# CERALIVE/ceracoder

Measured on AMD Instinct MI355X. Metric: 1080p H.264 encoded frames/sec per GPU, higher is better.
Workload: dtype u8

## Files before the change

ceracoder_amd/csrc/k_motion.hip:

```cpp
#include "kernels_common.hpp"

#ifndef ME_MBS
#define ME_MBS 4
#endif
#define ME_WQ (ME_MBS + 2)
#define ME_ROWS 50
#define ME_STRIDE 53
#define ME_K 5

DEV unsigned long long qsad(unsigned lo, unsigned hi, unsigned cur, unsigned long long acc) {
    unsigned long long src = ((unsigned long long)hi << 32) | lo;
    return __builtin_amdgcn_qsad_pk_u16_u8(src, cur, acc);
}
DEV int mv_bits(int v) {
    int a = iabs(v);
    return a == 0 ? 1 : 7 + 2 * (31 - __clz(a));
}
DEV int med3(int a, int b, int c) {
    const int lo = a < b ? a : b, hi = a < b ? b : a;
    return c < lo ? lo : (c > hi ? hi : c);
}
struct fpred_t { int px, py, sx, sy; };
DEV fpred_t field_pred(const imv_t *__restrict__ f, int mbw, int mx, int my, bool top) {
    const bool avA = mx > 0, avB = top, avC = top && mx + 1 < mbw, avD = mx > 0 && top, hasC = avC || avD;
// ... 146 lines not shown
#endif
#ifdef ME_DBG_NOSURF
    if (active && acc[0] == 0x123456789ull) {
#else
    if (active) {
#endif
        uint16_t *sf = ctx->surf + (size_t)(my * mbw + mx) * SURF_U16 + 4 * dxg;
#pragma unroll
        for (int d = 0; d < ME_K; d++) stg64(sf + (ME_K * g + d) * SURF_COLS, make_uint2((unsigned)acc[d], (unsigned)(acc[d] >> 32)));
    }
#ifdef ME_DBG_NOSEL
    const unsigned best = ((((unsigned)acc[0] ^ (unsigned)acc[4]) & 0x0FFFu) << 12) | 0x410u;
#else
    const unsigned best = select_min<true>(acc, g, dxg, active, ctx->me_range, ctx->lambda, 0, 0, 0, 0);
#endif
    if (lane == 0 && mx < mbw) store_imv(&ctx->imv_a[my * mbw + mx], best, ctx->lambda, 0, 0, 0, 0);
    tl_last(ctx, 1);
}

__global__ __launch_bounds__(256) void me_select_kernel(const frame_ctx_t cv, int mb0, int mb1, const imv_t *__restrict__ in, imv_t *__restrict__ out,
                                                        const imv_t *__restrict__ prev, int mode) {
    const frame_ctx_t *__restrict__ ctx = &cv;
    const int mbw = ctx->mbw;
    const int lane = threadIdx.x & 63, wave = __builtin_amdgcn_readfirstlane(threadIdx.x >> 6);
    const int mbn = mb0 + xcd_remap(blockIdx.x, gridDim.x) * 4 + wave;
    if (mbn >= mb1) return;
    const int my = mbn / mbw, mx = mbn - my * mbw;
    const fpred_t fp = field_pred(in, mbw, mx, my, row_has_top(ctx, my));
    const int px = fp.px >> 2, py = fp.py >> 2, sx = fp.sx >> 2, sy = fp.sy >> 2;
    if (mode) {
        fpred_t fq = {0, 0, 0, 0};
        if (mode == 2) fq = field_pred(prev, mbw, mx, my, row_has_top(ctx, my));
        if (px == (fq.px >> 2) && py == (fq.py >> 2) && sx == (fq.sx >> 2) && sy == (fq.sy >> 2)) {
            if (lane == 0) stg64(&out[mbn], ldg64(&in[mbn]));
            return;
        }
    }
    const bool active = lane < 63;
    const int g = active ? lane / 9 : 0, dxg = active ? lane % 9 : 0;
    unsigned long long acc[ME_K];
    const uint16_t *sf = ctx->surf + (size_t)mbn * SURF_U16 + 4 * dxg;
#pragma unroll
    for (int d = 0; d < ME_K; d++) { const uint2 v = ldg64(sf + (ME_K * g + d) * SURF_COLS); acc[d] = ((unsigned long long)v.y << 32) | v.x; }
    const unsigned best = select_min(acc, g, dxg, active, ctx->me_range, ctx->lambda, px, py, sx, sy);
    if (lane == 0) store_imv(&out[mbn], best, ctx->lambda, px, py, sx, sy);
}

#ifndef SEL_SPW
#define SEL_SPW 8
#endif
__global__ __launch_bounds__(256) void me_select_sparse_kernel(const frame_ctx_t cv, int mb0, int mb1, const imv_t *__restrict__ in, imv_t *__restrict__ out, const imv_t *__restrict__ prev) {
    const frame_ctx_t *__restrict__ ctx = &cv;
    const int mbw = ctx->mbw;
    const int lane = threadIdx.x & 63, wave = __builtin_amdgcn_readfirstlane(threadIdx.x >> 6);
    const int base = mb0 + ((int)blockIdx.x * 4 + wave) * SEL_SPW;
    if (base >= mb1) return;
    const int mine = base + (lane < SEL_SPW ? lane : 0);
    const bool have = lane < SEL_SPW && mine < mb1;
    const int mbn_l = have ? mine : base, my_l = mbn_l / mbw, mx_l = mbn_l - my_l * mbw;
    const bool top_l = row_has_top(ctx, my_l);
    const fpred_t fp = field_pred(in, mbw, mx_l, my_l, top_l), fq = field_pred(prev, mbw, mx_l, my_l, top_l);
    const int px = fp.px >> 2, py = fp.py >> 2, sx = fp.sx >> 2, sy = fp.sy >> 2;
    const bool same = px == (fq.px >> 2) && py == (fq.py >> 2) && sx == (fq.sx >> 2) && sy == (fq.sy >> 2);
    if (have && same) stg64(&out[mbn_l], ldg64(&in[mbn_l]));
    unsigned todo = (unsigned)(__ballot(have && !same) & ((1ull << SEL_SPW) - 1ull));
    const bool active = lane < 63;
    const int g = active ? lane / 9 : 0, dxg = active ? lane % 9 : 0;
    while (todo) {
        const int j = __builtin_ctz(todo);
        todo &= todo - 1;
        const int mbn = base + j;
        const int jpx = __builtin_amdgcn_readlane(px, j), jpy = __builtin_amdgcn_readlane(py, j), jsx = __builtin_amdgcn_readlane(sx, j), jsy = __builtin_amdgcn_readlane(sy, j);
        unsigned long long acc[ME_K];
        const uint16_t *sf = ctx->surf + (size_t)mbn * SURF_U16 + 4 * dxg;
#pragma unroll
        for (int d = 0; d < ME_K; d++) { const uint2 v = ldg64(sf + (ME_K * g + d) * SURF_COLS); acc[d] = ((unsigned long long)v.y << 32) | v.x; }
        const unsigned best = select_min(acc, g, dxg, active, ctx->me_range, ctx->lambda, jpx, jpy, jsx, jsy);
        if (lane == 0) store_imv(&out[mbn], best, ctx->lambda, jpx, jpy, jsx, jsy);
    }
}

#define SP_GS 24
#define SP_PS 20
struct sp_lds {
    uint8_t G[23 * SP_GS];
    int16_t H1[18 * SP_GS];
    uint8_t b[19 * SP_PS];
    uint8_t h[18 * SP_GS];
    uint8_t j[18 * SP_PS];
    uint8_t pad[16];
};
typedef short sp_s2 __attribute__((ext_vector_type(2)));
DEV sp_s2 as_s2(unsigned v) { return __builtin_bit_cast(sp_s2, v); }
DEV unsigned as_u(sp_s2 v) { return __builtin_bit_cast(unsigned, v); }
DEV sp_s2 bytes_lo(unsigned w) { return as_s2(__builtin_amdgcn_perm(0u, w, 0x0c010c00u)); }
DEV sp_s2 bytes_hi(unsigned w) { return as_s2(__builtin_amdgcn_perm(0u, w, 0x0c030c02u)); }
DEV sp_s2 clip255_s2(sp_s2 v) { return __builtin_elementwise_min(__builtin_elementwise_max(v, (sp_s2)(0)), (sp_s2)(255)); }
DEV sp_s2 pair_s2(int a, int b) { return as_s2(__builtin_amdgcn_perm((unsigned)b, (unsigned)a, 0x05040100u)); }
DEV unsigned pack_s2(sp_s2 lo, sp_s2 hi) { return __builtin_amdgcn_perm(as_u(hi), as_u(lo), 0x06040200u); }
DEV unsigned clip_pack4(int a, int b, int c, int d) { return pack_s2(clip255_s2(pair_s2(a, b)), clip255_s2(pair_s2(c, d))); }
DEV int mvq_bits(int q) {
    unsigned k = q > 0 ? (unsigned)(2 * q - 1) : (unsigned)(-2 * q);
    return 2 * (31 - __clz((int)(k + 1))) + 1;
}
DEV unsigned lds4(const uint8_t *plane, int o) {
    const unsigned *w = (const unsigned *)(plane + (o & ~3));
    return __builtin_amdgcn_alignbyte(w[1], w[0], (unsigned)(o & 3));
}
DEV unsigned sp_sample4(const sp_lds *L, int X, int Y, int fx, int fy) {
#define SG(x, y) lds4(L->G, ((y) + 2) * SP_GS + (x) + 2)
#define SB(x, y) lds4(L->b, (y) * SP_PS + (x))
#define SH(x, y) lds4(L->h, (y) * SP_GS + (x) + 2)
#define SJ(x, y) lds4(L->j, (y) * SP_PS + (x))
    if (fy == 0) {
        if (fx == 0) return SG(X, Y);
        return fx == 2 ? SB(X, Y) : fx == 1 ? avg4(SG(X, Y), SB(X, Y)) : avg4(SG(X + 1, Y), SB(X, Y));
    }
    if (fx == 0) return fy == 2 ? SH(X, Y) : fy == 1 ? avg4(SG(X, Y), SH(X, Y)) : avg4(SG(X, Y + 1), SH(X, Y));
    if ((fx & 1) && (fy & 1)) return avg4(fy == 1 ? SB(X, Y) : SB(X, Y + 1), fx == 1 ? SH(X, Y) : SH(X + 1, Y));
    if (fx == 2 && fy == 2) return SJ(X, Y);
    if (fx == 2) return avg4(fy == 1 ? SB(X, Y) : SB(X, Y + 1), SJ(X, Y));
    return avg4(fx == 1 ? SH(X, Y) : SH(X + 1, Y), SJ(X, Y));
#undef SG
#undef SB
#undef SH
#undef SJ
}
DEV void sp_planes(sp_lds *L, const int lane) {
    if (lane < 54) {
        const int d = lane % 6, seg = lane / 6;
        sp_s2 lo[7], hi[7];
#pragma unroll
        for (int r = 0; r < 7; r++) {
            const unsigned w = *(const unsigned *)&L->G[(2 * seg + r) * SP_GS + 4 * d];
            lo[r] = bytes_lo(w); hi[r] = bytes_hi(w);
        }
#pragma unroll
        for (int t = 0; t < 2; t++) {
            const sp_s2 vl = (lo[t + 2] + lo[t + 3]) * (sp_s2)(20) - (lo[t + 1] + lo[t + 4]) * (sp_s2)(5) + (lo[t] + lo[t + 5]);
            const sp_s2 vh = (hi[t + 2] + hi[t + 3]) * (sp_s2)(20) - (hi[t + 1] + hi[t + 4]) * (sp_s2)(5) + (hi[t] + hi[t + 5]);
            const int R = 2 * seg + t;
            unsigned *o = (unsigned *)&L->H1[R * SP_GS + 4 * d];
            o[0] = as_u(vl); o[1] = as_u(vh);
            *(unsigned *)&L->h[R * SP_GS + 4 * d] = pack_s2(clip255_s2((vl + (sp_s2)(16)) >> (sp_s2)(5)), clip255_s2((vh + (sp_s2)(16)) >> (sp_s2)(5)));
        }
    }
#pragma unroll
    for (int it = 0; it < 2; it++) {
        const int i = lane + 64 * it;
        if (i < 19 * 5) {
            const int R = i / 5, g = i - R * 5;
            const unsigned *gw = (const unsigned *)&L->G[(R + 2) * SP_GS + 4 * g];
            const unsigned d0 = gw[0] ^ 0x80808080u, d1 = gw[1] ^ 0x80808080u, d2 = gw[2] ^ 0x80808080u;
            int o[4];
#pragma unroll
            for (int k = 0; k < 4; k++) {
                const unsigned w0 = k ? __builtin_amdgcn_alignbyte(d1, d0, (unsigned)k) : d0, w1 = k ? __builtin_amdgcn_alignbyte(d2, d1, (unsigned)k) : d1;
                const int v = __builtin_amdgcn_sdot4((int)w0, 0x1414FB01, __builtin_amdgcn_sdot4((int)w1, 0x000001FB, 4096, false), false);
                o[k] = (v + 16) >> 5;
            }
            *(unsigned *)&L->b[R * SP_PS + 4 * g] = clip_pack4(o[0], o[1], o[2], o[3]);
        }
    }
    WAVE_SYNC();
#pragma unroll
    for (int it = 0; it < 2; it++) {
        const int i = lane + 64 * it;
        if (i < 18 * 5) {
            const int R = i / 5, g = i - R * 5;
            const unsigned *hw = (const unsigned *)&L->H1[R * SP_GS + 4 * g];
            const unsigned p0 = hw[0], p1 = hw[1], p2 = hw[2], p3 = hw[3], p4 = hw[4];
            const unsigned q0 = __builtin_amdgcn_alignbyte(p1, p0, 2u), q1 = __builtin_amdgcn_alignbyte(p2, p1, 2u),
                           q2 = __builtin_amdgcn_alignbyte(p3, p2, 2u), q3 = __builtin_amdgcn_alignbyte(p4, p3, 2u);
// ... 12 lines not shown
    const int mbw = ctx->mbw, mbh = ctx->mbh, stride = ctx->stride, W = mbw * 16, H = mbh * 16;
    const int lane = threadIdx.x & 63, wave = __builtin_amdgcn_readfirstlane(threadIdx.x >> 6);
    int mbn = mb0 + blockIdx.x * 4 + wave;
    const bool ok = mbn < mb1;
    if (!ok) mbn = mb1 - 1;
    const int my = mbn / mbw, mx = mbn - my * mbw, x0 = mx * 16, y0 = my * 16;
    sp_lds *L = &LD[wave];
    const mb_info_t info = ld_mbinfo(&ctx->mbi[mbn]);
    const int ix = x0 + (info.mvx >> 2), iy = y0 + (info.mvy >> 2);
    const uint8_t *__restrict__ ref = ctx->ref_y;
    if (ix - 3 >= 0 && iy - 3 >= 0 && ((ix - 3) & ~3) + 28 <= W && iy + 19 < H) {
        const int a = (ix - 3) & 3;
        const uint8_t *base = ref + (size_t)(iy - 3) * stride + ((ix - 3) & ~3);
        for (int i = lane; i < 23 * 6; i += 64) {
            const int r = i / 6, d = i - r * 6;
            const unsigned w0 = ldg32(base + (size_t)r * stride + 4 * d), w1 = ldg32(base + (size_t)r * stride + 4 * d + 4);
            *(unsigned *)&L->G[r * SP_GS + 4 * d] = __builtin_amdgcn_alignbyte(w1, w0, (unsigned)a);
        }
    } else
        for (int i = lane; i < 23 * 23; i += 64) {
            int r = i / 23, c = i - r * 23;
            int yy = clip3(0, H - 1, iy - 3 + r), xx = clip3(0, W - 1, ix - 3 + c);
            L->G[r * SP_GS + c] = (uint8_t)ldg8(ref + (size_t)yy * stride + xx);
        }
    const int pr = lane >> 2, pc = (lane & 3) * 4;
    unsigned curw;
    {
        int sy = y0 + pr;
        sy = sy < ctx->vis_h ? sy : ctx->vis_h - 1;
        curw = ldg32(ctx->src_y + (size_t)sy * ctx->src_stride + x0 + pc);
    }
    WAVE_SYNC();
    sp_planes(L, lane);
    const int lambda = ctx->lambda;
    int bqx = info.mvx, bqy = info.mvy;
    unsigned best = info.cost;
#pragma unroll 1
    for (int step = 2; step >= 1; step--) {
        const int cqx = bqx, cqy = bqy;
        unsigned acc[4] = {0, 0, 0, 0};
#pragma unroll
        for (int c8 = 0; c8 < 8; c8++) {
            const int k = c8 < 4 ? c8 : c8 + 1;
            const int qx = cqx + (k % 3 - 1) * step, qy = cqy + (k / 3 - 1) * step;
            const int ox = qx - info.mvx, oy = qy - info.mvy;
            const int X = 1 + (ox >> 2) + pc, Y = 1 + (oy >> 2) + pr;
            const unsigned sad = __builtin_amdgcn_sad_u8(curw, sp_sample4(L, X, Y, ox & 3, oy & 3), 0u);
            acc[c8 >> 1] |= sad << (16 * (c8 & 1));
        }
#pragma unroll
        for (int q = 0; q < 4; q++) {
            acc[q] = (unsigned)wave64_sum((int)acc[q]);
        }
#pragma unroll
        for (int c8 = 0; c8 < 8; c8++) {
            const int k = c8 < 4 ? c8 : c8 + 1;
            const int qx = cqx + (k % 3 - 1) * step, qy = cqy + (k / 3 - 1) * step;
            const unsigned sad = (acc[c8 >> 1] >> (16 * (c8 & 1))) & 0xFFFFu;
            const unsigned cost = sad + (unsigned)(lambda * (mvq_bits(qx) + mvq_bits(qy)));
            if (cost < best) { best = cost; bqx = qx; bqy = qy; }
        }
    }
    if (lane == 0 && ok) {
        mb_info_t *mb = &ctx->mbi[mbn];
        stg32(&mb->mvx, ((unsigned)(uint16_t)bqx) | ((unsigned)(uint16_t)bqy << 16));
        stg32(&mb->cost, best);
    }
}

DEV int dec_score(unsigned M) { return dec_score_mask(M); }
DEV int row_or4(int v) {
    v |= __builtin_amdgcn_update_dpp(0, v, 0x128, 0xF, 0xF, false);
    v |= __builtin_amdgcn_update_dpp(0, v, 0x124, 0xF, 0xF, false);
    return v;
}
DEV unsigned ref_word4(const uint8_t *__restrict__ ref, int stride, int W, int H, int x, int y, bool inside) {
    if (inside) {
        const uint8_t *b = ref + (size_t)y * stride + (x & ~3);
        return __builtin_amdgcn_alignbyte(ldg32(b + 4), ldg32(b), (unsigned)(x & 3));
    }
    const uint8_t *r = ref + (size_t)clip3(0, H - 1, y) * stride;
    return pack4((int)ldg8(r + clip3(0, W - 1, x)), (int)ldg8(r + clip3(0, W - 1, x + 1)), (int)ldg8(r + clip3(0, W - 1, x + 2)), (int)ldg8(r + clip3(0, W - 1, x + 3)));
}
DEV void chroma_pred4(const frame_ctx_t *__restrict__ ctx, int lane, int x0, int y0, int W, int H, int mvx, int mvy, int *pd) {
    const int stride = ctx->stride;
    const int py = (lane >> 2) & 3, cby = (lane >> 4) & 1, c = (lane >> 1) & 1, cbx = lane & 1;
    const int cx0 = x0 >> 1, cy0 = y0 >> 1, cw = W >> 1, ch = H >> 1;
    const int cy = cby * 4 + py, cxb = cbx * 4;
    const int xi = mvx >> 3, yi = mvy >> 3, xf = mvx & 7, yf = mvy & 7;
    const uint8_t *__restrict__ rf = ctx->ref_uv;
    int A[5], B[5];
    if (cx0 + xi >= 0 && cx0 + xi + 9 <= cw && cy0 + yi >= 0 && cy0 + yi + 9 <= ch) {
        const int o = 2 * (cx0 + cxb + xi) + c, a = o & 3;
        const uint8_t *r0 = rf + (size_t)(cy0 + cy + yi) * stride + (o & ~3), *r1 = r0 + stride;
        const unsigned a0 = ldg32(r0), a1 = ldg32(r0 + 4), a2 = ldg32(r0 + 8), b0 = ldg32(r1), b1 = ldg32(r1 + 4), b2 = ldg32(r1 + 8);
        const unsigned sa0 = __builtin_amdgcn_alignbyte(a1, a0, (unsigned)a), sa1 = __builtin_amdgcn_alignbyte(a2, a1, (unsigned)a);
        const unsigned sb0 = __builtin_amdgcn_alignbyte(b1, b0, (unsigned)a), sb1 = __builtin_amdgcn_alignbyte(b2, b1, (unsigned)a);
        A[0] = byte_of(sa0, 0); A[1] = byte_of(sa0, 2); A[2] = byte_of(sa1, 0); A[3] = byte_of(sa1, 2); A[4] = (int)((a2 >> (8 * a)) & 255);
        B[0] = byte_of(sb0, 0); B[1] = byte_of(sb0, 2); B[2] = byte_of(sb1, 0); B[3] = byte_of(sb1, 2); B[4] = (int)((b2 >> (8 * a)) & 255);
    } else {
        const int ya = clip3(0, ch - 1, cy0 + cy + yi), yb = clip3(0, ch - 1, cy0 + cy + yi + 1);
#pragma unroll
        for (int i = 0; i < 5; i++) {
            const int xx = clip3(0, cw - 1, cx0 + cxb + i + xi);
            A[i] = (int)ldg8(rf + (size_t)ya * stride + 2 * xx + c);
            B[i] = (int)ldg8(rf + (size_t)yb * stride + 2 * xx + c);
        }
    }
    const int w00 = (8 - xf) * (8 - yf), w10 = xf * (8 - yf), w01 = (8 - xf) * yf, w11 = xf * yf;
#pragma unroll
    for (int i = 0; i < 4; i++) pd[i] = (w00 * A[i] + w10 * A[i + 1] + w01 * B[i] + w11 * B[i + 1] + 32) >> 6;
}
DEV unsigned pmb_luma_tq(const dev_tables *T, int lane, unsigned curw, unsigned pw, int qp, bool decimate, int *lev, int *x) {
    const int py = (lane >> 2) & 3, fy = ((py & 1) << 1) | (py >> 1);
    const col_bf cb = make_col_bf(py);
    const int kz0 = (int)((0xFEA9DB83C7426510ull >> (16 * fy)) & 0xFFFF);
    const qparams q = make_q(T, qp, false);
    const int mfe = py < 2 ? q.mf[0] : q.mf[2], mfo = py < 2 ? q.mf[2] : q.mf[1], ve = py < 2 ? q.v[0] : q.v[2], vo = py < 2 ? q.v[2] : q.v[1];
#pragma unroll
    for (int i = 0; i < 4; i++) x[i] = byte_of(curw, i) - byte_of(pw, i);
    fwd_rows4(x);
    unsigned m = 0, big = 0;
#pragma unroll
    for (int i = 0; i < 4; i++) {
        const int cf = fwd_col(x[i], cb);
        lev[i] = quant1(cf, (i & 1) ? mfo : mfe, q.f, q.qbits);
        m |= (lev[i] != 0 ? 1u : 0u) << ((kz0 >> (4 * i)) & 15);
        big |= (lev[i] > 1 || lev[i] < -1) ? 1u : 0u;
    }
    if (decimate) {
        const unsigned mm = (unsigned)row_or4((int)(m | (big << 16)));
        int s = (mm >> 16) ? 9 : dec_score(((mm & 0xFFFFu) << 1) | 1u);
        int s8 = s + quad_xor<1>(s);
        s8 += __shfl_xor(s8, 16, 64);
        int tot = s8 + quad_xor<2>(s8);
        tot += __shfl_xor(tot, 32, 64);
        if (s8 < 4 || tot < 6) { lev[0] = lev[1] = lev[2] = lev[3] = 0; }
    }
#pragma unroll
    for (int i = 0; i < 4; i++) x[i] = (lev[i] * ((i & 1) ? vo : ve)) << q.shift;
    const unsigned long long bal = __ballot((lev[0] | lev[1] | lev[2] | lev[3]) != 0);
    const unsigned long long t = bal | (bal >> 4) | (bal >> 8) | (bal >> 12);
    const int rb = lane & 15, rbx = blkx(rb) >> 2, rby = blky(rb) >> 2;
    return (unsigned)(__ballot(lane < 16 && ((t >> (16 * rby + rbx)) & 1)) & 0xFFFFull);
}
DEV unsigned pmb_satd(int lane, unsigned curw, unsigned pw) {
    const int py = (lane >> 2) & 3, s1 = py < 2 ? 1 : -1, s2 = (py & 1) ? -1 : 1;
    const int d0 = byte_of(curw, 0) - byte_of(pw, 0), d1 = byte_of(curw, 1) - byte_of(pw, 1), d2 = byte_of(curw, 2) - byte_of(pw, 2), d3 = byte_of(curw, 3) - byte_of(pw, 3);
    const int a = d0 + d3, b = d1 + d2, c = d1 - d2, e = d0 - d3;
    int t[4] = {a + b, e + c, a - b, e - c};
    int acc = 0;
#pragma unroll
    for (int i = 0; i < 4; i++) {
        const int u = mad24(t[i], s1, row_xor8(t[i]));
        const int w = mad24(u, s2, row_xor4(u));
        acc += iabs(w);
    }
    return (unsigned)wave64_sum(acc);
}
DEV unsigned pmb_sa8d(int lane, unsigned curw, unsigned pw) {
    const int s0 = (lane & 1) ? -1 : 1, s1 = (lane & 4) ? -1 : 1, s2 = (lane & 8) ? -1 : 1, s3 = (lane & 16) ? -1 : 1;
    const int d0 = byte_of(curw, 0) - byte_of(pw, 0), d1 = byte_of(curw, 1) - byte_of(pw, 1), d2 = byte_of(curw, 2) - byte_of(pw, 2), d3 = byte_of(curw, 3) - byte_of(pw, 3);
    const int a = d0 + d3, b = d1 + d2, c = d1 - d2, e = d0 - d3;
    int t[4] = {a + b, e + c, a - b, e - c};
    int acc = 0;
#pragma unroll
    for (int i = 0; i < 4; i++) {
        int u = mad24(t[i], s0, quad_xor<1>(t[i]));
        u = mad24(u, s1, row_xor4(u));
        u = mad24(u, s2, row_xor8(u));
        u = mad24(u, s3, __shfl_xor(u, 16, 64));
        acc += iabs(u);
    }
    return (unsigned)wave64_sum(acc);
}
DEV bool pmb_pick_t8(int lane, unsigned curw, unsigned pw) {
    const unsigned raw4 = pmb_satd(lane, curw, pw), raw8 = pmb_sa8d(lane, curw, pw);
    return __builtin_amdgcn_readfirstlane((int)(((raw8 + 2) >> 2) < (raw4 >> 1))) != 0;
}
template <bool SC1>
DEV void pmb_store_pred_only(const frame_ctx_t *__restrict__ ctx, int16_t *lv, int lane, int x0, int y0, unsigned pw, const int *pd) {
    const int stride = ctx->stride, pr = lane >> 2, pc = (lane & 3) * 4;
    stx32<SC1>(ctx->rec_y + (size_t)(y0 + pr) * stride + x0 + pc, pw);
    const int py = (lane >> 2) & 3, cby = (lane >> 4) & 1, c = (lane >> 1) & 1, cbx = lane & 1;
    const unsigned mine = pack4(pd[0], pd[1], pd[2], pd[3]), other = (unsigned)quad_xor<2>((int)mine);
    if (lane < 32 && c == 0) {
        uint2 out;
        out.x = __builtin_amdgcn_perm(other, mine, 0x05010400u);
        out.y = __builtin_amdgcn_perm(other, mine, 0x07030602u);
        stx64<SC1>(ctx->rec_uv + (size_t)((y0 >> 1) + cby * 4 + py) * stride + 2 * ((x0 >> 1) + cbx * 4), out);
    }
    if (lane < MB_LEVELS * 2 / 16) stg128(lv + 8 * lane, make_uint4(0, 0, 0, 0));
}

template <bool SC1>
DEV unsigned pmb_luma_t8(const frame_ctx_t *__restrict__ ctx, int *tile, int lane, unsigned curw, unsigned pw, int qp, int mbn, int x0, int y0) {
    const int pr = lane >> 2, pc = (lane & 3) * 4;
    {
        int *t = tile + ((pr >> 3) * 2 + (pc >> 3)) * 64 + (pr & 7) * 8 + (pc & 7);
#pragma unroll
        for (int i = 0; i < 4; i++) t[i] = byte_of(curw, i) - byte_of(pw, i);
    }
    WAVE_SYNC();
    const bool act = lane < 16;
    const int i8 = (lane >> 2) & 3, j = lane & 3;
    int *tb = tile + i8 * 64;
    const int m6 = qp % 6, k6 = qp / 6;
    int rs[2][8], cw[2][8];
    unsigned submask = 0;
    if (act) {
#pragma unroll
        for (int r = 0; r < 2; r++) {
#pragma unroll
            for (int i = 0; i < 8; i++) rs[r][i] = tb[(2 * j + r) * 8 + i];
            fdct8_1d(rs[r]);
        }
    }
    WAVE_SYNC();
    if (act) {
#pragma unroll
        for (int r = 0; r < 2; r++)
#pragma unroll
            for (int i = 0; i < 8; i++) tb[(2 * j + r) * 8 + i] = rs[r][i];
    }
    WAVE_SYNC();
    if (act) {
#pragma unroll
        for (int c2 = 0; c2 < 2; c2++) {
#pragma unroll
            for (int r = 0; r < 8; r++) cw[c2][r] = tb[r * 8 + 2 * j + c2];
            fdct8_1d(cw[c2]);
#pragma unroll
            for (int r = 0; r < 8; r++) {
                const int xx = 2 * j + c2, cl = pos_class8(r, xx);
                const int qbits = 16 + k6, f = (1 << qbits) / 6;
                const int a = iabs(cw[c2][r]);
                int l = (int)(((long long)a * g_tab.mf8[m6][cl] + f) >> qbits);
                l = l > 2047 ? 2047 : l;
                l = cw[c2][r] < 0 ? -l : l;
                const int kk = g_tab.izz8[r * 8 + xx];
                stg16(&ctx->levels[(size_t)mbn * MB_LEVELS + L_LUMA + (4 * i8 + (kk & 3)) * 16 + (kk >> 2)], l);
                if (l) submask |= 1u << (kk & 3);
// ... 59 lines not shown
    v += (unsigned)row_xor8((int)v);
    v += (unsigned)__shfl_xor((int)v, 16, 64);
    return v;
}
DEV unsigned part_total(unsigned g) { g += (unsigned)quad_xor<2>((int)g); return g + (unsigned)__shfl_xor((int)g, 32, 64); }
#ifdef PMB_PROF
#define PMB_NPH 11
#define PMB_MARK(k) do { const unsigned long long t1_ = __builtin_readcyclecounter(); ph_[k] = t1_ - t0_; t0_ = t1_; } while (0)
#define PMB_MARK0() unsigned long long ph_[PMB_NPH] = {0, 0, 0, 0, 0, 0, 0, 0, 0, 0, 0}; unsigned long long t0_ = __builtin_readcyclecounter()
#define PMB_FLUSH() do { if (lane == 0) for (int k_ = 0; k_ < PMB_NPH; k_++) stg32((unsigned *)ctx->dbrec + (size_t)mbn * 16 + k_, (unsigned)ph_[k_]); } while (0)
#else
#define PMB_MARK(k) ((void)0)
#define PMB_MARK0() ((void)0)
#define PMB_FLUSH() ((void)0)
#endif
struct pmb_pre_t { uint2 selfw; fpred_t fp; unsigned curw; uint2 sw; unsigned ds; uint4 dw; };
DEV pmb_pre_t pmb_preload(const frame_ctx_t *__restrict__ ctx, const int mbn, const int lane) {
    const int mbw = ctx->mbw, my = mbn / mbw, mx = mbn - my * mbw, x0 = mx * 16, y0 = my * 16;
    pmb_pre_t p;
    const imv_t *__restrict__ field = k_final_imv_dev(ctx);
    p.selfw = ldg64(field + mbn);
    {
        int sy = y0 + (lane >> 2);
        sy = sy < ctx->vis_h ? sy : ctx->vis_h - 1;
        p.curw = ldg32(ctx->src_y + (size_t)sy * ctx->src_stride + x0 + (lane & 3) * 4);
    }
    {
        const int cby = (lane >> 4) & 1, cbx = lane & 1;
        int sy = (y0 >> 1) + cby * 4 + ((lane >> 2) & 3);
        const int vh2 = ctx->vis_h >> 1;
        sy = sy < vh2 ? sy : vh2 - 1;
        p.sw = ldg64(ctx->src_uv + (size_t)sy * ctx->src_stride + 2 * ((x0 >> 1) + cbx * 4));
    }
    p.dw = ctx->intra_p ? ldg128(ctx->idec + (size_t)mbn * IDEC_BYTES + 16) : make_uint4(0, 0, 0, 0);
    p.fp = field_pred(field, mbw, mx, my, row_has_top(ctx, my));
    p.ds = (unsigned)*(const GAS uint16_t *)(ctx->surf + (size_t)mbn * SURF_U16 + ((p.fp.sy >> 2) + 16) * SURF_COLS + (p.fp.sx >> 2) + 16);
    return p;
}
DEV bool ir_ok(const frame_ctx_t *__restrict__ ctx, int mx, int mvx) {
    return mx >= ctx->ir_c0 || (16 * mx + 15 + (mvx >> 2) + ((mvx & 3) ? 3 : 0) <= ctx->ir_clean && 8 * mx + 7 + (mvx >> 3) + ((mvx & 7) ? 1 : 0) <= (ctx->ir_clean >> 1));
}
DEV int ir_max_whole(const frame_ctx_t *__restrict__ ctx, int mx) {
    const int kl = ctx->ir_clean - 16 * mx - 15, kc = 2 * ((ctx->ir_clean >> 1) - 8 * mx - 7);
    return 4 * (kl < kc ? kl : kc);
}
template <bool SC1>
DEV void pmb_store_intra(mb_info_t *mb, const uint4 dw, int qp, int lane) {
    if (lane == 0) {
        const bool i4 = ((dw.x >> 16) & 255u) != 0;
        mb_info_t m;
        m.mvx = 0; m.mvy = 0; m.mb_type = i4 ? 2 : 0; m.i16_mode = i4 ? 0 : (uint8_t)(dw.x & 255u); m.chroma_mode = (uint8_t)((dw.x >> 8) & 255u);
        m.qp = (uint8_t)qp; m.nzmask = 0; m.cost = dw.y;
        st_mbinfo_x<SC1>(mb, m);
    }
}
template <bool SC1, bool PART, int T8, bool IR>
DEV void pmb_mb(const frame_ctx_t *__restrict__ ctx, sp_lds *L, const int mbn, const int lane, const int refine, const pmb_pre_t &pre) {
    const int mbw = ctx->mbw, mbh = ctx->mbh, stride = ctx->stride, W = mbw * 16, H = mbh * 16, qp = mb_qp_dev(ctx, mbn), lambda = ctx->lambda;
    const int my = mbn / mbw, mx = mbn - my * mbw, x0 = mx * 16, y0 = my * 16;
    const dev_tables *T = &g_tab;
    PMB_MARK0();
    const uint2 selfw = pre.selfw;
    int imx = (int)(int16_t)(selfw.x & 0xFFFF);
    const int imy = (int)(int16_t)(selfw.x >> 16);
    const unsigned di = selfw.y & 0xFFFFu, ibits = selfw.y >> 16;
    const fpred_t fp = pre.fp;
    const int pr = lane >> 2, pc = (lane & 3) * 4;
    const int py = (lane >> 2) & 3;
    const unsigned curw = pre.curw;
    int sv[4];
    {
        const int c = (lane >> 1) & 1;
        const uint2 sw = pre.sw;
        const unsigned slo = c ? (sw.x >> 8) : sw.x, shi = c ? (sw.y >> 8) : sw.y;
        sv[0] = (int)(slo & 255); sv[1] = (int)((slo >> 16) & 255); sv[2] = (int)(shi & 255); sv[3] = (int)((shi >> 16) & 255);
    }
    int16_t *lv = ctx->levels + (size_t)mbn * MB_LEVELS;
    mb_info_t *mb = &ctx->mbi[mbn];
    if (IR && mx >= ctx->ir_c0 && mx < ctx->ir_c1) {
        pmb_store_intra<SC1>(mb, pre.dw, qp, lane);
        PMB_FLUSH();
        return;
    }
    {
        const unsigned ds = pre.ds;
        const bool skip_ok = !IR || ir_ok(ctx, mx, fp.sx);
        bool pass = ctx->drop_sad && ds < ctx->drop_sad && skip_ok;
        const bool worth = ds <= di + (unsigned)(lambda * SKIP_MARGIN_BITS) && skip_ok;
        PMB_MARK(0);
        if (pass || worth) {
            const int X = x0 + (fp.sx >> 2), Y = y0 + (fp.sy >> 2);
            const bool inside = X >= 0 && Y >= 0 && X + 16 <= W && Y + 16 <= H;
            const unsigned pw = ref_word4(ctx->ref_y, stride, W, H, X + pc, Y + pr, inside);
            int pd[4];
            chroma_pred4(ctx, lane, x0, y0, W, H, fp.sx, fp.sy, pd);
            if (!pass) {
                int lev[4], x[4];
                if (pmb_luma_tq(T, lane, curw, pw, qp, true, lev, x) == 0) {
                    unsigned nz_c = 0, dc_c = 0;
                    chroma_rows4(ctx, T, lv, x0 >> 1, y0 >> 1, lane, pd, sv, qp, false, false, nullptr, nz_c, dc_c, true, 0, SC1);
                    pass = (nz_c | dc_c) == 0;
                }
            }
            PMB_MARK(1);
            if (pass) {
                pmb_store_pred_only<SC1>(ctx, lv, lane, x0, y0, pw, pd);
                if (lane == 0) {
                    mb_info_t m;
                    m.mvx = (int16_t)fp.sx; m.mvy = (int16_t)fp.sy; m.mb_type = 1; m.i16_mode = 0; m.chroma_mode = 0; m.qp = (uint8_t)qp; m.nzmask = 0; m.cost = di;
                    st_mbinfo_x<SC1>(mb, m);
                }
                PMB_FLUSH();
                return;
            }
        }
    }
    if (IR && !ir_ok(ctx, mx, imx)) imx = ir_max_whole(ctx, mx);
    const int ix = x0 + (imx >> 2), iy = y0 + (imy >> 2);
    const uint8_t *__restrict__ ref = ctx->ref_y;
    if (ix - 3 >= 0 && iy - 3 >= 0 && ((ix - 3) & ~3) + 28 <= W && iy + 19 < H) {
        const int a = (ix - 3) & 3;
        const uint8_t *base = ref + (size_t)(iy - 3) * stride + ((ix - 3) & ~3);
        for (int i = lane; i < 23 * 6; i += 64) {
            const int r = i / 6, d = i - r * 6;
            const unsigned w0 = ldg32(base + (size_t)r * stride + 4 * d), w1 = ldg32(base + (size_t)r * stride + 4 * d + 4);
            *(unsigned *)&L->G[r * SP_GS + 4 * d] = __builtin_amdgcn_alignbyte(w1, w0, (unsigned)a);
        }
    } else
        for (int i = lane; i < 23 * 23; i += 64) {
            int r = i / 23, c = i - r * 23;
            int yy = clip3(0, H - 1, iy - 3 + r), xx = clip3(0, W - 1, ix - 3 + c);
            L->G[r * SP_GS + c] = (uint8_t)ldg8(ref + (size_t)yy * stride + xx);
        }
    WAVE_SYNC();
    PMB_MARK(2);
    int bqx = imx, bqy = imy;
    unsigned q0 = 0, qh[4] = {0, 0, 0, 0}, qq[4] = {0, 0, 0, 0};
    int hbx = imx, hby = imy;
    unsigned best;
    if (PART) {
        q0 = part_gsum(__builtin_amdgcn_sad_u8(curw, sp_sample4(L, 1 + pc, 1 + pr, 0, 0), 0u));
        best = part_total(q0) + (unsigned)(lambda * (mvq_bits(imx - fp.px) + mvq_bits(imy - fp.py)));
    } else
        best = (unsigned)wave64_sum((int)__builtin_amdgcn_sad_u8(curw, sp_sample4(L, 1 + pc, 1 + pr, 0, 0), 0u)) +
               (unsigned)(lambda * (mvq_bits(imx - fp.px) + mvq_bits(imy - fp.py)));
    PMB_MARK(3);
    if (refine) {
        sp_planes(L, lane);
        PMB_MARK(4);
        {
            const int cqx = bqx, cqy = bqy;
            unsigned acc[4] = {0, 0, 0, 0};
#pragma unroll
            for (int c8 = 0; c8 < 8; c8++) {
                const int k = c8 < 4 ? c8 : c8 + 1;
                const int qx = cqx + (k % 3 - 1) * 2, qy = cqy + (k / 3 - 1) * 2;
                const int ox = qx - imx, oy = qy - imy;
                const unsigned sad = __builtin_amdgcn_sad_u8(curw, sp_sample4(L, 1 + (ox >> 2) + pc, 1 + (oy >> 2) + pr, ox & 3, oy & 3), 0u);
                acc[c8 >> 1] |= sad << (16 * (c8 & 1));
            }
#pragma unroll
            for (int q = 0; q < 4; q++) {
                if (PART) { qh[q] = part_gsum(acc[q]); acc[q] = part_total(qh[q]); }
                else acc[q] = (unsigned)wave64_sum((int)acc[q]);
            }
#pragma unroll
            for (int c8 = 0; c8 < 8; c8++) {
                const int k = c8 < 4 ? c8 : c8 + 1;
                const int qx = cqx + (k % 3 - 1) * 2, qy = cqy + (k / 3 - 1) * 2;
                const unsigned sad = (acc[c8 >> 1] >> (16 * (c8 & 1))) & 0xFFFFu;
                const unsigned cost = sad + (unsigned)(lambda * (mvq_bits(qx - fp.px) + mvq_bits(qy - fp.py)));
                if (cost < best && (!IR || ir_ok(ctx, mx, qx))) { best = cost; bqx = qx; bqy = qy; }
            }
        }
        hbx = bqx; hby = bqy;
        PMB_MARK(5);
        {
            const int cqx = bqx, cqy = bqy;
            {
                const int ox = cqx - imx, oy = cqy - imy;
                best = (pmb_satd(lane, curw, sp_sample4(L, 1 + (ox >> 2) + pc, 1 + (oy >> 2) + pr, ox & 3, oy & 3)) >> 1) +
                       (unsigned)(lambda * (mvq_bits(cqx - fp.px) + mvq_bits(cqy - fp.py)));
            }
#pragma unroll 1
            for (int k = 0; k < 9; k++) {
                if (k == 4) continue;
                const int qx = cqx + (k % 3 - 1), qy = cqy + (k / 3 - 1);
                const int ox = qx - imx, oy = qy - imy;
                const unsigned cw = sp_sample4(L, 1 + (ox >> 2) + pc, 1 + (oy >> 2) + pr, ox & 3, oy & 3);
                if (PART) {
                    const int c8 = k < 4 ? k : k - 1;
                    const unsigned g = part_gsum(__builtin_amdgcn_sad_u8(curw, cw, 0u)) << (16 * (c8 & 1));
                    qq[0] |= (c8 >> 1) == 0 ? g : 0u; qq[1] |= (c8 >> 1) == 1 ? g : 0u; qq[2] |= (c8 >> 1) == 2 ? g : 0u; qq[3] |= (c8 >> 1) == 3 ? g : 0u;
                }
                const unsigned d = pmb_satd(lane, curw, cw) >> 1;
                const unsigned cost = d + (unsigned)(lambda * (mvq_bits(qx - fp.px) + mvq_bits(qy - fp.py)));
                if (cost < best && (!IR || ir_ok(ctx, mx, qx))) { best = cost; bqx = qx; bqy = qy; }
            }
        }
    }
    PMB_MARK(6);
    const int ox = bqx - imx, oy = bqy - imy;
    unsigned pw = sp_sample4(L, 1 + (ox >> 2) + pc, 1 + (oy >> 2) + pr, ox & 3, oy & 3);
    unsigned dsad = (unsigned)wave64_sum((int)__builtin_amdgcn_sad_u8(curw, pw, 0u));
    unsigned jinter = dsad + (unsigned)(lambda * (mvq_bits(bqx - fp.px) + mvq_bits(bqy - fp.py)));
    int shape = 0, lvx = bqx, lvy = bqy;
    if (PART && refine) {
        unsigned k8 = 0xFFFFFFFFu, k168 = 0xFFFFFFFFu, k816 = 0xFFFFFFFFu;
#pragma unroll 1
        for (int k = 0; k < 17; k++) {
            const int cx = k == 0 ? imx : k < 9 ? imx + (((k - 1 < 4 ? k - 1 : k) % 3) - 1) * 2 : hbx + (((k - 9 < 4 ? k - 9 : k - 8) % 3) - 1);
            const int cy = k == 0 ? imy : k < 9 ? imy + (((k - 1 < 4 ? k - 1 : k) / 3) - 1) * 2 : hby + (((k - 9 < 4 ? k - 9 : k - 8) / 3) - 1);
            const unsigned bits = (unsigned)(lambda * (mvq_bits(cx - fp.px) + mvq_bits(cy - fp.py)));
            const int c8 = k == 0 ? 0 : k < 9 ? k - 1 : k - 9;
            const unsigned pk = k == 0 ? q0 : k < 9 ? ((c8 >> 1) == 0 ? qh[0] : (c8 >> 1) == 1 ? qh[1] : (c8 >> 1) == 2 ? qh[2] : qh[3])
                                                    : ((c8 >> 1) == 0 ? qq[0] : (c8 >> 1) == 1 ? qq[1] : (c8 >> 1) == 2 ? qq[2] : qq[3]);
            const unsigned sq = k == 0 ? pk : (pk >> (16 * (c8 & 1))) & 0xFFFFu;
            const unsigned sh = sq + (unsigned)quad_xor<2>((int)sq);
            const unsigned sv_ = sq + (unsigned)__shfl_xor((int)sq, 32, 64);
            const unsigned a = ((sq + bits) << 5) | (unsigned)k, b = ((sh + bits) << 5) | (unsigned)k, c = ((sv_ + bits) << 5) | (unsigned)k;
            k8 = a < k8 ? a : k8; k168 = b < k168 ? b : k168; k816 = c < k816 ? c : k816;
        }
        const unsigned c8x8 = (k8 >> 5), c168 = (k168 >> 5), c816 = (k816 >> 5);
        unsigned t8 = c8x8 + (unsigned)quad_xor<2>((int)c8x8); t8 += (unsigned)__shfl_xor((int)t8, 32, 64);
        const unsigned t168 = c168 + (unsigned)__shfl_xor((int)c168, 32, 64);
        const unsigned t816 = c816 + (unsigned)quad_xor<2>((int)c816);
        unsigned jb = jinter + (unsigned)lambda;
        unsigned key = 0;
        const unsigned j1 = t168 + 3u * (unsigned)lambda, j2 = t816 + 3u * (unsigned)lambda, j3 = t8 + 9u * (unsigned)lambda;
        if (j1 < jb) { jb = j1; shape = 1; key = k168; }
        if (j2 < jb) { jb = j2; shape = 2; key = k816; }
        if (j3 < jb) { jb = j3; shape = 3; key = k8; }
        shape = __builtin_amdgcn_readfirstlane(shape);
        if (shape) {
            const int k = (int)(key & 31u);
            lvx = k == 0 ? imx : k < 9 ? imx + (((k - 1 < 4 ? k - 1 : k) % 3) - 1) * 2 : hbx + (((k - 9 < 4 ? k - 9 : k - 8) % 3) - 1);
            lvy = k == 0 ? imy : k < 9 ? imy + (((k - 1 < 4 ? k - 1 : k) / 3) - 1) * 2 : hby + (((k - 9 < 4 ? k - 9 : k - 8) / 3) - 1);
            const int px_ = lvx - imx, py_ = lvy - imy;
            pw = sp_sample4(L, 1 + (px_ >> 2) + pc, 1 + (py_ >> 2) + pr, px_ & 3, py_ & 3);
            dsad = (unsigned)wave64_sum((int)__builtin_amdgcn_sad_u8(curw, pw, 0u));
            jinter = jb - (unsigned)lambda;
        }
    }
    if (ctx->intra_p && di + (unsigned)lambda * ibits >= INTRA_GATE(lambda)) {
        const uint4 dw = pre.dw;
        const unsigned jintra = dw.z + (dw.z >> 3) + (unsigned)(lambda * 12);
        if (jintra < jinter) {
            pmb_store_intra<SC1>(mb, dw, qp, lane);
            PMB_FLUSH();
            return;
        }
    }
    PMB_MARK(7);
    int pd[4];
    unsigned slot = 0;
    if (PART && shape) {
        const int src = (((lane >> 4) & 1) << 5) | ((lane & 1) << 1);
        const int cvx = __shfl(lvx, src, 64), cvy = __shfl(lvy, src, 64);
        chroma_pred4(ctx, lane, x0, y0, W, H, cvx, cvy, pd);
        const unsigned mine = ((unsigned)(uint16_t)lvx) | ((unsigned)(uint16_t)lvy << 16);
        const unsigned v1 = (unsigned)__shfl((int)mine, shape == 1 ? 32 : 2, 64), v2 = (unsigned)__shfl((int)mine, 32, 64), v3 = (unsigned)__shfl((int)mine, 34, 64);
        slot = lane == 0 ? v1 : (shape == 3 && lane == 1) ? v2 : (shape == 3 && lane == 2) ? v3 : 0u;
        bqx = __builtin_amdgcn_readfirstlane(lvx); bqy = __builtin_amdgcn_readfirstlane(lvy);
    } else chroma_pred4(ctx, lane, x0, y0, W, H, bqx, bqy, pd);
    if (ctx->drop_sad && dsad < ctx->drop_sad) {
        pmb_store_pred_only<SC1>(ctx, lv, lane, x0, y0, pw, pd);
        if (PART && shape && lane < 8) stx32<SC1>(lv + L_LDC + 2 * lane, slot);
        if (lane == 0) {
            mb_info_t m;
            m.mvx = (int16_t)bqx; m.mvy = (int16_t)bqy; m.mb_type = 1; m.i16_mode = (uint8_t)shape; m.chroma_mode = 0; m.qp = (uint8_t)qp; m.nzmask = 0; m.cost = di;
            st_mbinfo_x<SC1>(mb, m);
        }
        PMB_FLUSH();
        return;
    }
    PMB_MARK(8);
    unsigned nz_luma;
    const bool t8 = T8 == 1 || (T8 == 2 && pmb_pick_t8(lane, curw, pw));
    if (t8) {
        nz_luma = pmb_luma_t8<SC1>(ctx, (int *)L, lane, curw, pw, qp, mbn, x0, y0);
    } else {
        const int fy = ((py & 1) << 1) | (py >> 1);
        const col_bf cb = make_col_bf(py);
        const int kz0 = (int)((0xFEA9DB83C7426510ull >> (16 * fy)) & 0xFFFF);
        int lev[4], x[4];
        nz_luma = pmb_luma_tq(T, lane, curw, pw, qp, true, lev, x);
        const int bx = lane & 3, by = lane >> 4, b = ((by >> 1) << 3) | ((bx >> 1) << 2) | ((by & 1) << 1) | (bx & 1);
#pragma unroll
        for (int i = 0; i < 4; i++) stg16(&lv[L_LUMA + b * 16 + ((kz0 >> (4 * i)) & 15)], lev[i]);
        inv_rows4(x);
        int o[4];
#pragma unroll
        for (int i = 0; i < 4; i++) o[i] = clip255(byte_of(pw, i) + ((inv_col(x[i], cb) + 32) >> 6));
        stx32<SC1>(ctx->rec_y + (size_t)(y0 + pr) * stride + x0 + pc, pack4(o[0], o[1], o[2], o[3]));
    }
    PMB_MARK(9);
    unsigned nz_c = 0, dc_c = 0;
    chroma_rows4(ctx, T, lv, x0 >> 1, y0 >> 1, lane, pd, sv, qp, false, true, nullptr, nz_c, dc_c, true, 0, SC1);
    PMB_MARK(10);
    if (lane == 0) {
        unsigned nzm = nz_luma | (nz_c << 16);
        if (dc_c & 1) nzm |= NZ_CBDC;
        if (dc_c & 2) nzm |= NZ_CRDC;
        if (t8 && nz_luma) nzm |= NZ_T8;
        mb_info_t m;
        m.mvx = (int16_t)bqx; m.mvy = (int16_t)bqy; m.mb_type = 1; m.i16_mode = (uint8_t)shape; m.chroma_mode = 0; m.qp = (uint8_t)qp; m.nzmask = nzm; m.cost = di;
        st_mbinfo_x<SC1>(mb, m);
    }
    if (PART && shape) { if (lane < 8) stx32<SC1>(lv + L_LDC + 2 * lane, slot); }
    else if (lane < 2) stg128(lv + L_LDC + 8 * lane, make_uint4(0, 0, 0, 0));
    PMB_FLUSH();
}

template <bool GATED, bool ROWS, bool PART, int T8, bool IR = false>
__global__ __launch_bounds__(256) void pmb_kernel(const frame_ctx_t cv, int mb0, int mb1, int refine, const unsigned *__restrict__ gate_done, unsigned ref_epoch, unsigned *err, unsigned *row_done) {
    const frame_ctx_t *__restrict__ ctx = &cv;
    __shared__ __attribute__((aligned(16))) sp_lds LD[4];
    const int lane = threadIdx.x & 63, wave = __builtin_amdgcn_readfirstlane(threadIdx.x >> 6);
    const int mbn = mb0 + 4 * (int)blockIdx.x + wave;
    if (mb0 == 0 && blockIdx.x == 0) tl_first(ctx, 2);
    pmb_pre_t pre;
    if (mbn < mb1) pre = pmb_preload(ctx, mbn, lane);
    if (GATED) {
        if (wave == 0) {
            const int mbw = ctx->mbw, mbh = ctx->mbh;
            const int first = mb0 + 4 * (int)blockIdx.x, last = first + 3 < mb1 ? first + 3 : mb1 - 1;
            int r_lo = first / mbw - 2, r_hi = last / mbw + 2;
            r_lo = r_lo > 0 ? r_lo : 0;
            r_hi = r_hi < mbh ? r_hi : mbh - 1;
            const uint2 *flags = (const uint2 *)(gate_done + DB_DONE_STRIDE * (blockIdx.x & (DB_DONE_COPIES - 1)));
            const int b_hi = r_hi / MI355_BAND_ROWS;
#ifdef DBG_OLD_GATE
            int spins = 0, b = b_hi;
#else
            int spins = 0, b = r_lo / MI355_BAND_ROWS;
#endif
            for (;;) {
                const uint2 f = ld64_sc1(flags + b);
                if (f.x == ref_epoch && f.y == ref_epoch) { if (++b > b_hi) break; continue; }
#ifndef PMB_POLL_SLEEP
#define PMB_POLL_SLEEP 64
#endif
                __builtin_amdgcn_s_sleep(PMB_POLL_SLEEP);
                if (++spins > DB_SPIN_MAX) { st_sc1(err, 3u); break; }
                if ((spins & 255) == 0 && ld_sc1(err)) break;
            }
            __builtin_amdgcn_fence(__ATOMIC_ACQUIRE, "agent");
// ... 100 lines not shown
```

Baseline: 7438.

## Prefetch luma search window and chroma neighborhood into LDS before skip probe

```diff
diff --git a/ceracoder_amd/csrc/k_motion.hip b/ceracoder_amd/csrc/k_motion.hip
--- a/ceracoder_amd/csrc/k_motion.hip
+++ b/ceracoder_amd/csrc/k_motion.hip
@@ -252,6 +252,7 @@
 
 #define SP_GS 24
 #define SP_PS 20
+#define SP_CW 6
 struct sp_lds {
     uint8_t G[23 * SP_GS];
     int16_t H1[18 * SP_GS];
@@ -259,6 +260,7 @@
     uint8_t h[18 * SP_GS];
     uint8_t j[18 * SP_PS];
     uint8_t pad[16];
+    unsigned C[10 * SP_CW];
 };
 typedef short sp_s2 __attribute__((ext_vector_type(2)));
 DEV sp_s2 as_s2(unsigned v) { return __builtin_bit_cast(sp_s2, v); }
@@ -437,6 +439,11 @@
     const uint8_t *r = ref + (size_t)clip3(0, H - 1, y) * stride;
     return pack4((int)ldg8(r + clip3(0, W - 1, x)), (int)ldg8(r + clip3(0, W - 1, x + 1)), (int)ldg8(r + clip3(0, W - 1, x + 2)), (int)ldg8(r + clip3(0, W - 1, x + 3)));
 }
+DEV void chroma_bilinear4(const int *A, const int *B, int xf, int yf, int *pd) {
+    const int w00 = (8 - xf) * (8 - yf), w10 = xf * (8 - yf), w01 = (8 - xf) * yf, w11 = xf * yf;
+#pragma unroll
+    for (int i = 0; i < 4; i++) pd[i] = (w00 * A[i] + w10 * A[i + 1] + w01 * B[i] + w11 * B[i + 1] + 32) >> 6;
+}
 DEV void chroma_pred4(const frame_ctx_t *__restrict__ ctx, int lane, int x0, int y0, int W, int H, int mvx, int mvy, int *pd) {
     const int stride = ctx->stride;
     const int py = (lane >> 2) & 3, cby = (lane >> 4) & 1, c = (lane >> 1) & 1, cbx = lane & 1;
@@ -462,9 +469,56 @@
             B[i] = (int)ldg8(rf + (size_t)yb * stride + 2 * xx + c);
         }
     }
-    const int w00 = (8 - xf) * (8 - yf), w10 = xf * (8 - yf), w01 = (8 - xf) * yf, w11 = xf * yf;
-#pragma unroll
-    for (int i = 0; i < 4; i++) pd[i] = (w00 * A[i] + w10 * A[i + 1] + w01 * B[i] + w11 * B[i + 1] + 32) >> 6;
+    chroma_bilinear4(A, B, xf, yf, pd);
+}
+DEV bool pmb_win_inside(int W, int H, int ix, int iy) { return ix - 3 >= 0 && iy - 3 >= 0 && ((ix - 3) & ~3) + 28 <= W && iy + 19 < H; }
+DEV bool pmb_cnb_inside(int W, int H, int X0, int Y0) { return X0 >= 0 && X0 + 10 <= (W >> 1) && Y0 >= 0 && Y0 + 10 <= (H >> 1); }
+struct pmb_ref_t { unsigned w0, w1, w2, w3, w4, w5, c0; };
+DEV pmb_ref_t pmb_ref_issue(const frame_ctx_t *__restrict__ ctx, sp_lds *L, int lane, int W, int H, int ix, int iy, int X0, int Y0) {
+    const int stride = ctx->stride;
+    const uint8_t *__restrict__ ref = ctx->ref_y;
+    pmb_ref_t r = {0, 0, 0, 0, 0, 0, 0};
+    if (pmb_win_inside(W, H, ix, iy)) {
+        const int base = (iy - 3) * stride + ((ix - 3) & ~3);
+        const int i0 = lane, i1 = lane + 64, i2 = lane + 128 < 23 * 6 ? lane + 128 : 23 * 6 - 1;
+        const unsigned o0 = (unsigned)(base + (i0 / 6) * stride + 4 * (i0 % 6)), o1 = (unsigned)(base + (i1 / 6) * stride + 4 * (i1 % 6)),
+                       o2 = (unsigned)(base + (i2 / 6) * stride + 4 * (i2 % 6));
+        r.w0 = ldg32(ref + o0); r.w1 = ldg32(ref + o0 + 4); r.w2 = ldg32(ref + o1); r.w3 = ldg32(ref + o1 + 4); r.w4 = ldg32(ref + o2); r.w5 = ldg32(ref + o2 + 4);
+    } else
+        for (int i = lane; i < 23 * 23; i += 64) {
+            int rr = i / 23, c = i - rr * 23;
+            int yy = clip3(0, H - 1, iy - 3 + rr), xx = clip3(0, W - 1, ix - 3 + c);
+            L->G[rr * SP_GS + c] = (uint8_t)ldg8(ref + (size_t)yy * stride + xx);
+        }
+    const uint8_t *__restrict__ rf = ctx->ref_uv;
+    if (pmb_cnb_inside(W, H, X0, Y0)) {
+        const int l = lane < 10 * SP_CW ? lane : 0, rr = l / SP_CW, d = l - rr * SP_CW, ca = (2 * X0) & 3;
+        r.c0 = ldg32(rf + (unsigned)((Y0 + rr) * stride + ((2 * X0) & ~3) + 4 * ((d < 5 || ca) ? d : 0)));
+    } else if (lane < 50) {
+        const int rr = lane / 5, d = lane - rr * 5;
+        const uint8_t *row = rf + (size_t)clip3(0, (H >> 1) - 1, Y0 + rr) * stride;
+        const int xa = clip3(0, (W >> 1) - 1, X0 + 2 * d), xb = clip3(0, (W >> 1) - 1, X0 + 2 * d + 1);
+        L->C[rr * SP_CW + d] = pack4((int)ldg8(row + 2 * xa), (int)ldg8(row + 2 * xa + 1), (int)ldg8(row + 2 * xb), (int)ldg8(row + 2 * xb + 1));
+    }
+    return r;
+}
+DEV void pmb_ref_store(sp_lds *L, int lane, int W, int H, int ix, int iy, int X0, int Y0, const pmb_ref_t r) {
+    if (pmb_win_inside(W, H, ix, iy)) {
+        const unsigned a = (unsigned)((ix - 3) & 3);
+        const int i0 = lane, i1 = lane + 64, i2 = lane + 128;
+        *(unsigned *)&L->G[(i0 / 6) * SP_GS + 4 * (i0 % 6)] = __builtin_amdgcn_alignbyte(r.w1, r.w0, a);
+        *(unsigned *)&L->G[(i1 / 6) * SP_GS + 4 * (i1 % 6)] = __builtin_amdgcn_alignbyte(r.w3, r.w2, a);
+        if (i2 < 23 * 6) *(unsigned *)&L->G[(i2 / 6) * SP_GS + 4 * (i2 % 6)] = __builtin_amdgcn_alignbyte(r.w5, r.w4, a);
+    }
+    if (pmb_cnb_inside(W, H, X0, Y0) && lane < 10 * SP_CW && (lane % SP_CW < 5 || ((2 * X0) & 3))) L->C[lane] = r.c0;
+}
+DEV void chroma_pred4_lds(const sp_lds *L, int lane, int cxr, int cyr, int ca, int mvx, int mvy, int *pd) {
+    const int py = (lane >> 2) & 3, cby = (lane >> 4) & 1, c = (lane >> 1) & 1, cbx = lane & 1;
+    const uint8_t *p = (const uint8_t *)L->C + (cby * 4 + py + (mvy >> 3) - cyr) * (4 * SP_CW) + ca + 2 * (cbx * 4 + (mvx >> 3) - cxr) + c;
+    int A[5], B[5];
+#pragma unroll
+    for (int i = 0; i < 5; i++) { A[i] = (int)p[2 * i]; B[i] = (int)p[4 * SP_CW + 2 * i]; }
+    chroma_bilinear4(A, B, mvx & 7, mvy & 7, pd);
 }
 DEV unsigned pmb_luma_tq(const dev_tables *T, int lane, unsigned curw, unsigned pw, int qp, bool decimate, int *lev, int *x) {
     const int py = (lane >> 2) & 3, fy = ((py & 1) << 1) | (py >> 1);
@@ -499,7 +553,7 @@
     const int rb = lane & 15, rbx = blkx(rb) >> 2, rby = blky(rb) >> 2;
     return (unsigned)(__ballot(lane < 16 && ((t >> (16 * rby + rbx)) & 1)) & 0xFFFFull);
 }
-DEV unsigned pmb_satd(int lane, unsigned curw, unsigned pw) {
+DEV int pmb_satd_lane(int lane, unsigned curw, unsigned pw) {
     const int py = (lane >> 2) & 3, s1 = py < 2 ? 1 : -1, s2 = (py & 1) ? -1 : 1;
     const int d0 = byte_of(curw, 0) - byte_of(pw, 0), d1 = byte_of(curw, 1) - byte_of(pw, 1), d2 = byte_of(curw, 2) - byte_of(pw, 2), d3 = byte_of(curw, 3) - byte_of(pw, 3);
     const int a = d0 + d3, b = d1 + d2, c = d1 - d2, e = d0 - d3;
@@ -511,8 +565,9 @@
         const int w = mad24(u, s2, row_xor4(u));
         acc += iabs(w);
     }
-    return (unsigned)wave64_sum(acc);
-}
+    return acc;
+}
+DEV unsigned pmb_satd(int lane, unsigned curw, unsigned pw) { return (unsigned)wave64_sum(pmb_satd_lane(lane, curw, pw)); }
 DEV unsigned pmb_sa8d(int lane, unsigned curw, unsigned pw) {
     const int s0 = (lane & 1) ? -1 : 1, s1 = (lane & 4) ? -1 : 1, s2 = (lane & 8) ? -1 : 1, s3 = (lane & 16) ? -1 : 1;
     const int d0 = byte_of(curw, 0) - byte_of(pw, 0), d1 = byte_of(curw, 1) - byte_of(pw, 1), d2 = byte_of(curw, 2) - byte_of(pw, 2), d3 = byte_of(curw, 3) - byte_of(pw, 3);
@@ -738,58 +793,56 @@
         PMB_FLUSH();
         return;
     }
-    {
-        const unsigned ds = pre.ds;
-        const bool skip_ok = !IR || ir_ok(ctx, mx, fp.sx);
-        bool pass = ctx->drop_sad && ds < ctx->drop_sad && skip_ok;
-        const bool worth = ds <= di + (unsigned)(lambda * SKIP_MARGIN_BITS) && skip_ok;
-        PMB_MARK(0);
-        if (pass || worth) {
-            const int X = x0 + (fp.sx >> 2), Y = y0 + (fp.sy >> 2);
-            const bool inside = X >= 0 && Y >= 0 && X + 16 <= W && Y + 16 <= H;
-            const unsigned pw = ref_word4(ctx->ref_y, stride, W, H, X + pc, Y + pr, inside);
-            int pd[4];
-            chroma_pred4(ctx, lane, x0, y0, W, H, fp.sx, fp.sy, pd);
-            if (!pass) {
-                int lev[4], x[4];
-                if (pmb_luma_tq(T, lane, curw, pw, qp, true, lev, x) == 0) {
-                    unsigned nz_c = 0, dc_c = 0;
-                    chroma_rows4(ctx, T, lv, x0 >> 1, y0 >> 1, lane, pd, sv, qp, false, false, nullptr, nz_c, dc_c, true, 0, SC1);
-                    pass = (nz_c | dc_c) == 0;
-                }
-            }
-            PMB_MARK(1);
-            if (pass) {
-                pmb_store_pred_only<SC1>(ctx, lv, lane, x0, y0, pw, pd);
-                if (lane == 0) {
-                    mb_info_t m;
-                    m.mvx = (int16_t)fp.sx; m.mvy = (int16_t)fp.sy; m.mb_type = 1; m.i16_mode = 0; m.chroma_mode = 0; m.qp = (uint8_t)qp; m.nzmask = 0; m.cost = di;
-                    st_mbinfo_x<SC1>(mb, m);
-                }
-                PMB_FLUSH();
-                return;
-            }
-        }
-    }
+    const unsigned ds = pre.ds;
+    const bool skip_ok = !IR || ir_ok(ctx, mx, fp.sx);
+    bool pass = ctx->drop_sad && ds < ctx->drop_sad && skip_ok;
+    const bool worth = ds <= di + (unsigned)(lambda * SKIP_MARGIN_BITS) && skip_ok;
+    const bool probe = pass || worth;
     if (IR && !ir_ok(ctx, mx, imx)) imx = ir_max_whole(ctx, mx);
     const int ix = x0 + (imx >> 2), iy = y0 + (imy >> 2);
-    const uint8_t *__restrict__ ref = ctx->ref_y;
-    if (ix - 3 >= 0 && iy - 3 >= 0 && ((ix - 3) & ~3) + 28 <= W && iy + 19 < H) {
-        const int a = (ix - 3) & 3;
-        const uint8_t *base = ref + (size_t)(iy - 3) * stride + ((ix - 3) & ~3);
-        for (int i = lane; i < 23 * 6; i += 64) {
-            const int r = i / 6, d = i - r * 6;
-            const unsigned w0 = ldg32(base + (size_t)r * stride + 4 * d), w1 = ldg32(base + (size_t)r * stride + 4 * d + 4);
-            *(unsigned *)&L->G[r * SP_GS + 4 * d] = __builtin_amdgcn_alignbyte(w1, w0, (unsigned)a);
-        }
-    } else
-        for (int i = lane; i < 23 * 23; i += 64) {
-            int r = i / 23, c = i - r * 23;
-            int yy = clip3(0, H - 1, iy - 3 + r), xx = clip3(0, W - 1, ix - 3 + c);
-            L->G[r * SP_GS + c] = (uint8_t)ldg8(ref + (size_t)yy * stride + xx);
-        }
-    WAVE_SYNC();
-    PMB_MARK(2);
+    const int cxr = (imx >> 3) - 1, cyr = (imy >> 3) - 1, X0 = (x0 >> 1) + cxr, Y0 = (y0 >> 1) + cyr;
+    const int ca = pmb_cnb_inside(W, H, X0, Y0) ? ((2 * X0) & 3) : 0;
+#ifndef PMB_WIN_EARLY
+#define PMB_WIN_EARLY 1
+#endif
+    const bool early = PMB_WIN_EARLY || !probe;
+    const int SX = x0 + (fp.sx >> 2), SY = y0 + (fp.sy >> 2);
+    const bool inside = SX >= 0 && SY >= 0 && SX + 16 <= W && SY + 16 <= H;
+    PMB_MARK(0);
+    pmb_ref_t rr = {0, 0, 0, 0, 0, 0, 0};
+    if (early) rr = pmb_ref_issue(ctx, L, lane, W, H, ix, iy, X0, Y0);
+    if (probe) {
+        const unsigned pw = ref_word4(ctx->ref_y, stride, W, H, SX + pc, SY + pr, inside);
+        int pd[4];
+        chroma_pred4(ctx, lane, x0, y0, W, H, fp.sx, fp.sy, pd);
+        if (early) pmb_ref_store(L, lane, W, H, ix, iy, X0, Y0, rr);
+        PMB_MARK(2);
+        if (!pass) {
+            int lev[4], x[4];
+            if (pmb_luma_tq(T, lane, curw, pw, qp, true, lev, x) == 0) {
+                unsigned nz_c = 0, dc_c = 0;
+                chroma_rows4(ctx, T, lv, x0 >> 1, y0 >> 1, lane, pd, sv, qp, false, false, nullptr, nz_c, dc_c, true, 0, SC1);
+                pass = (nz_c | dc_c) == 0;
+            }
+        }
+        PMB_MARK(1);
+        if (pass) {
+            pmb_store_pred_only<SC1>(ctx, lv, lane, x0, y0, pw, pd);
+            if (lane == 0) {
+                mb_info_t m;
+                m.mvx = (int16_t)fp.sx; m.mvy = (int16_t)fp.sy; m.mb_type = 1; m.i16_mode = 0; m.chroma_mode = 0; m.qp = (uint8_t)qp; m.nzmask = 0; m.cost = di;
+                st_mbinfo_x<SC1>(mb, m);
+            }
+            PMB_FLUSH();
+            return;
+        }
+    }
+    if (!probe || !early) {
+        if (!early) rr = pmb_ref_issue(ctx, L, lane, W, H, ix, iy, X0, Y0);
+        pmb_ref_store(L, lane, W, H, ix, iy, X0, Y0, rr);
+        PMB_MARK(2);
+    }
+    WAVE_SYNC();
     int bqx = imx, bqy = imy;
     unsigned q0 = 0, qh[4] = {0, 0, 0, 0}, qq[4] = {0, 0, 0, 0};
     int hbx = imx, hby = imy;
@@ -913,12 +966,12 @@
     if (PART && shape) {
         const int src = (((lane >> 4) & 1) << 5) | ((lane & 1) << 1);
         const int cvx = __shfl(lvx, src, 64), cvy = __shfl(lvy, src, 64);
-        chroma_pred4(ctx, lane, x0, y0, W, H, cvx, cvy, pd);
+        chroma_pred4_lds(L, lane, cxr, cyr, ca, cvx, cvy, pd);
         const unsigned mine = ((unsigned)(uint16_t)lvx) | ((unsigned)(uint16_t)lvy << 16);
         const unsigned v1 = (unsigned)__shfl((int)mine, shape == 1 ? 32 : 2, 64), v2 = (unsigned)__shfl((int)mine, 32, 64), v3 = (unsigned)__shfl((int)mine, 34, 64);
         slot = lane == 0 ? v1 : (shape == 3 && lane == 1) ? v2 : (shape == 3 && lane == 2) ? v3 : 0u;
         bqx = __builtin_amdgcn_readfirstlane(lvx); bqy = __builtin_amdgcn_readfirstlane(lvy);
-    } else chroma_pred4(ctx, lane, x0, y0, W, H, bqx, bqy, pd);
+    } else chroma_pred4_lds(L, lane, cxr, cyr, ca, bqx, bqy, pd);
     if (ctx->drop_sad && dsad < ctx->drop_sad) {
         pmb_store_pred_only<SC1>(ctx, lv, lane, x0, y0, pw, pd);
         if (PART && shape && lane < 8) stx32<SC1>(lv + L_LDC + 2 * lane, slot);
```

Result: no change. 7413 (-0.3%).
